# ironhide23586/RoomNet

Hardware: AMD Instinct MI355X
Metric: images/sec, 224x224 batch-256 RoomNet inference (higher is better)
Workload: dtype bf16; 1 GPU; RoomNet forward (reference final_model weights), uint8 BGR 224x224x3 in HBM -> probs+ids in HBM, batch 256 per GPU, bf16 storage / fp32 accumulate; images_per_gpu=256, global_batch=256, im_side=224, parallelism=dp1

## Files before the change

roomnet_amd/csrc/rn_stage4x.hip:

```cpp
#include "rn_fused.h"
#include "rn_stage.h"

#include <utility>

using namespace rnk;

namespace {

constexpr int U_NS = 4;
constexpr int U_AHEAD = 3;
constexpr int U_RINGPX = 208;
constexpr int U_ROW = U_RINGPX * 64;
constexpr int U_TAB_BYTES = 4 * 64 * 4;
constexpr int U_RING_OFF = U_TAB_BYTES;
constexpr int U_LDS = U_RING_OFF + U_NS * U_ROW;
constexpr int U_WMIN = 193, U_WMAX = 206;

template <int DT, int NQ>
__global__ __launch_bounds__(NQ == 4 ? 512 : 768, NQ == 4 ? 2 : 3) void stage4x_kernel(const StageArgs a) {
    constexpr int U_NW = NQ == 4 ? 8 : 12;
    constexpr int U_NTH = U_NW * 64;
    constexpr int U_NT = NQ == 4 ? 7 : 4;
    constexpr int U_NU = (U_NT + 1) / 2;
    RN_CLOCK_ENTRY();
    extern __shared__ __attribute__((aligned(64))) char smem[];
    const int tid = threadIdx.x;
    const int lane = tid & 63;
    const int wave = __builtin_amdgcn_readfirstlane(tid >> 6);
    const int cq = NQ == 4 ? (wave & 3) : (wave >> 2);
    const int run = NQ == 4 ? (wave >> 2) : (((wave & 3) + (wave >> 2)) & 3);
    const int px16 = lane & 15, g = lane >> 4;
    const int cb = blockIdx.x % a.n_cb, band = blockIdx.x / a.n_cb, n = blockIdx.y;
    const int Win = a.W, Wo_full = a.Wo, Ho = a.Ho;
    const int xo0 = a.cb_xo0[cb], Wo = a.cb_wo[cb];
    const int x0 = 2 * xo0;
    const int W = min(2 * Wo + 4, Win - x0);
    const int yo0 = band * a.rows_per_band;
    const int nrows = min(Ho, yo0 + a.rows_per_band) - yo0;
    const int y0 = 2 * yo0;
    const int nconv = 2 * (nrows - 1) + 4;
    const int nin = nconv + 2;
    const f32x4 zero4 = {0.f, 0.f, 0.f, 0.f};
    constexpr int OOB = 0x40000000;

    char* const ring = smem + U_RING_OFF;
    const unsigned ring_lds = lds_addr(ring);
    for (int i = tid; i < U_NS * (U_RINGPX - U_WMIN) * 4; i += U_NTH) {
        const int slot = i / ((U_RINGPX - U_WMIN) * 4), rest = i % ((U_RINGPX - U_WMIN) * 4);
        const int p = U_WMIN + rest / 4, c = rest % 4;
        if (p >= W) *reinterpret_cast<i32x4*>(ring + slot * U_ROW + p * 64 + c * 16) = i32x4{0, 0, 0, 0};
    }

    const bool has7 = run == 0;
    const int xo_run = NQ == 4 ? (run ? 55 : 0) : (run ? 8 + 23 * run : 0);
    const int xw = 2 * xo_run;
    const int nout_run = NQ == 4 ? (has7 ? 55 : 47) : (has7 ? 31 : 23);

    i32x4 wf[9];
#pragma unroll
    for (int f = 0; f < 9; ++f) {
        const i32x4* src = a.wfrag + (f * 4 + cq) * 64 + lane;
        asm volatile("global_load_dwordx4 %0, %1, off" : "=v"(wf[f]) : "v"(src) : "memory");
    }

    const char* const in_img = reinterpret_cast<const char*>(a.in + static_cast<int64_t>(n) * Win * Win * 32) + x0 * 64;
    const int row_bytes = Win * 64;
    const unsigned goff0 = static_cast<unsigned>((tid >> 2) * 64 + (((tid & 3) ^ swz4x(tid >> 2)) << 4));
    const int tail_total = W * 4 - U_NTH;
    const int tailn = (tail_total + U_NW - 1) / U_NW;
    const int tail_start = min(wave * tailn, tail_total - 1);
    const int tail_cnt = max(1, min(tail_total - wave * tailn, tailn));
    const unsigned long long tail_mask = (1ull << tail_cnt) - 1ull;
    unsigned goff1;
    {
        const int q = U_NTH + tail_start + min(lane, tail_cnt - 1);
        const int p = q >> 2, c = q & 3;
        goff1 = static_cast<unsigned>(p * 64 + ((c ^ swz4x(p)) << 4));
    }
    auto issue_row = [&](int y, int slot) __attribute__((always_inline)) {
        const char* row = in_img + static_cast<int64_t>(y0 + min(y, nin - 1)) * row_bytes;
        unsigned o0 = goff0, o1 = goff1;
        asm volatile("" : "+v"(o0), "+v"(o1));
        dma16(row + o0, ring + slot * U_ROW + wave * 1024);
        dma16_masked(row + o1, ring + slot * U_ROW + (U_NTH + tail_start) * 16, tail_mask);
    };

    unsigned base[3];
#pragma unroll
    for (int kx = 0; kx < 3; ++kx) {
        const int p = xw + px16 + kx;
        base[kx] = ring_lds + static_cast<unsigned>(p * 64 + ((g ^ swz4x(p)) << 4));
    }

    RN_POOL_BANDS_S2(pmA, pmB, pmC, px16, g);

    int voff[U_NU];
#pragma unroll
    for (int u = 0; u < U_NU; ++u) {
        const int xo = xo_run + 16 * u + px16;
        const bool valid = 16 * u + px16 < nout_run && xo < Wo;
        voff[u] = valid ? ((xo0 + xo) * 64 + 16 * cq + 4 * g) * 2 : OOB;
    }
    [[maybe_unused]] i32x2 cq3v = {0, 0};
    if constexpr (NQ == 3) cq3v = *reinterpret_cast<const i32x2*>(a.cvals + 4 * g);
    const f32x4 sc = *reinterpret_cast<const f32x4*>(a.ptab + 16 * cq + 4 * g);
    const f32x4 sh = *reinterpret_cast<const f32x4*>(a.ptab + 64 + 16 * cq + 4 * g);

    f32x4 acc[3][U_NT];
    int hp[U_NT][2], pp2[U_NT][2];
#pragma unroll
    for (int k = 0; k < U_NT; ++k) {
        hp[k][0] = hp[k][1] = pp2[k][0] = pp2[k][1] = 0;
#pragma unroll
        for (int r3 = 0; r3 < 3; ++r3) acc[r3][k] = zero4;
    }
    const int out_row_bytes = Wo_full * 128;
    const char* const out_img = reinterpret_cast<const char*>(a.out + static_cast<int64_t>(n) * Ho * Wo_full * 64);

#pragma unroll
    for (int j = 0; j < U_AHEAD; ++j) issue_row(j, j);
    wait_vmcnt<0>();
#pragma unroll
    for (int f = 0; f < 9; ++f) asm volatile("" : "+v"(wf[f]));
    lds_barrier();

    int slot_cur = 0;
    i32x4 fq[2][3];
    auto reads_at = [&](auto KC, const unsigned (&bcr)[3]) __attribute__((always_inline)) {
        constexpr int k = decltype(KC)::value;
        auto& dst = fq[k & 1];
#pragma unroll
        for (int f = 0; f < 3; ++f) asm volatile("ds_read_b128 %0, %1 offset:%2" : "=v"(dst[f]) : "v"(bcr[f]), "n"(k * 1024));
    };
    {
        unsigned bc0[3] = {base[0], base[1], base[2]};
        reads_at(IC<0>{}, bc0);
    }
    auto step = [&](auto RC, auto PARC, int s) __attribute__((always_inline)) {
        constexpr int R = decltype(RC)::value, PAR = decltype(PARC)::value;
        constexpr int iN = R, iM = (R + 2) % 3, iO = (R + 1) % 3;
        wait_vmcnt<(NQ == 4 ? 5 : 4)>();
        raw_barrier();
        const unsigned so = static_cast<unsigned>(slot_cur * U_ROW);
        unsigned bc[3];
#pragma unroll
        for (int kx = 0; kx < 3; ++kx) bc[kx] = base[kx] + so;
        i32x4 op[U_NT + 1];
        op[U_NT - 1] = op[U_NT] = i32x4{0, 0, 0, 0};
        auto reads = [&](auto KC) __attribute__((always_inline)) { reads_at(KC, bc); };
        auto tile = [&](auto KC, auto NEXTC) __attribute__((always_inline)) {
            constexpr int k = decltype(KC)::value;
            constexpr bool NEXT = decltype(NEXTC)::value != 0;
            if constexpr (NEXT) reads(IC<k + 1>{});
            auto& cur = fq[k & 1];
            [&]<int... F>(std::integer_sequence<int, F...>) {
                (([&] {
                     asm volatile("s_waitcnt lgkmcnt(%1)" : "+v"(cur[F]) : "n"((NEXT ? 3 : 0) + 2 - F));
                     acc[iN][k] = mfma16<DT>(cur[F], wf[0 * 3 + F], F == 0 ? zero4 : acc[iN][k]);
                     acc[iM][k] = mfma16<DT>(cur[F], wf[1 * 3 + F], acc[iM][k]);
                     acc[iO][k] = mfma16<DT>(cur[F], wf[2 * 3 + F], acc[iO][k]);
                     if constexpr (k == 0 && F == 0) {
                         int sl = slot_cur + U_AHEAD;
                         sl = sl >= U_NS ? sl - U_NS : sl;
                         issue_row(s + U_AHEAD, sl);
                     }
                 }()),
                 ...);
            }(std::make_integer_sequence<int, 3>{});
            const f32x4 v = acc[iO][k];
            const int v0 = static_cast<int>(pack2_relu6_sixth(v[0], v[1]));
            const int v1 = static_cast<int>(pack2_relu6_sixth(v[2], v[3]));
            if constexpr (PAR == 0) {
                hp[k][0] = v0;
                hp[k][1] = v1;
            } else {
                const int n0 = pk_add_f16(hp[k][0], v0), n1 = pk_add_f16(hp[k][1], v1);
                op[k] = i32x4{pp2[k][0], pp2[k][1], n0, n1};
                pp2[k][0] = n0;
                pp2[k][1] = n1;
            }
        };
        [&]<int... K>(std::integer_sequence<int, K...>) {
            (tile(IC<K>{}, IC<(K + 2 < U_NT ? 1 : 0)>{}), ...);
        }(std::make_integer_sequence<int, U_NT - 1>{});
        if (has7) {
            reads(IC<U_NT - 1>{});
            tile(IC<U_NT - 1>{}, IC<0>{});
        }
        if constexpr (PAR == 1) {
            const int r = (s - 5) >> 1;
            const bool emit = s >= 5 && r < nrows;
            const int rr = min(max(r, 0), nrows - 1);
            const char* orow = out_img + static_cast<int64_t>(yo0 + rr) * out_row_bytes;
            const __amdgpu_buffer_rsrc_t rs = __builtin_amdgcn_make_buffer_rsrc(const_cast<char*>(orow), 0, out_row_bytes, 0x00020000);
            const int emask = emit ? 0 : OOB;
            [[maybe_unused]] const unsigned seed = (!a.dither || cq == a.plain_q) ? RN_SEED_PLAIN : rn_dither_seed(yo0 + rr);
            auto out = [&](auto UC) __attribute__((always_inline)) {
                constexpr int u = decltype(UC)::value;
                f32x4 H = mfma16<RN_DTYPE_F16>(op[2 * u], pmA, zero4);
                H = mfma16<RN_DTYPE_F16>(op[2 * u + 1], pmB, H);
                if constexpr (2 * u + 2 < U_NT) H = mfma16<RN_DTYPE_F16>(op[2 * u + 2], pmC, H);
                float y[4];
#pragma unroll
                for (int i = 0; i < 4; ++i) y[i] = __builtin_fmaf(H[i], sc[i], sh[i]);
                i32x2 d;
                if constexpr (DT == RN_DTYPE_BF16)
                    d = i32x2{static_cast<int>(pack2_sr_bf16(y[0], y[1], seed)), static_cast<int>(pack2_sr_bf16(y[2], y[3], seed))};
                else
                    d = i32x2{static_cast<int>(pack2<DT>(y[0], y[1])), static_cast<int>(pack2<DT>(y[2], y[3]))};
                __builtin_amdgcn_raw_buffer_store_b64(d, rs, voff[u] | emask, 0, 0);
                if constexpr (NQ == 3)
                    if (cq == 2) __builtin_amdgcn_raw_buffer_store_b64(cq3v, rs, (voff[u] + 32) | emask, 0, 0);
            };
            if constexpr (NQ == 4) {
                out(IC<0>{});
                out(IC<1>{});
                out(IC<2>{});
                if (has7) out(IC<3>{});
            } else {
                out(IC<0>{});
                out(IC<1>{});
            }
        }
        slot_cur = slot_cur == U_NS - 1 ? 0 : slot_cur + 1;
        asm volatile("s_waitcnt lgkmcnt(0)" ::: "memory");
        {
            const unsigned sn = static_cast<unsigned>(slot_cur * U_ROW);
            unsigned bn[3];
#pragma unroll
            for (int kx = 0; kx < 3; ++kx) bn[kx] = base[kx] + sn;
            reads_at(IC<0>{}, bn);
        }
    };
    int s = 0;
    for (; s + 5 < nin; s += 6) {
        step(IC<0>{}, IC<0>{}, s);
        step(IC<1>{}, IC<1>{}, s + 1);
        step(IC<2>{}, IC<0>{}, s + 2);
        step(IC<0>{}, IC<1>{}, s + 3);
        step(IC<1>{}, IC<0>{}, s + 4);
        step(IC<2>{}, IC<1>{}, s + 5);
    }
    const int rem = nin - s;
    if (rem > 0) step(IC<0>{}, IC<0>{}, s);
    if (rem > 1) step(IC<1>{}, IC<1>{}, s + 1);
    if (rem > 2) step(IC<2>{}, IC<0>{}, s + 2);
    if (rem > 3) step(IC<0>{}, IC<1>{}, s + 3);
    if (rem > 4) step(IC<1>{}, IC<0>{}, s + 4);
    wait_vmcnt<0>();
    RN_CLOCK_EXIT(a.stamp_buf, threadIdx.x == 256);
}

}

bool rn_stage4x_plan(int out_side, int* n_cb, int* xo0, int* wo) {
    return rn_colblock_plan(out_side, (U_WMIN + 1 - 4 + 1) / 2, (U_WMAX - 4) / 2, n_cb, xo0, wo);
}

bool rn_stage4x_supported(int cin, int cout, int pool_k, int pool_s, bool res, int in_side) {
    int ncb, xo0[4], wo[4];
    return cin == 32 && cout == 64 && pool_k == 4 && pool_s == 2 && !res && in_side >= U_WMIN &&
           rn_stage4x_plan((in_side - 6) / 2 + 1, &ncb, xo0, wo);
}

void rn_stage4x_pack(const float* w_hwio, int dtype, std::vector<unsigned short>* out) {
    out->assign(static_cast<size_t>(9) * 4 * 64 * 8, 0);
    for (int f = 0; f < 9; ++f)
        for (int q = 0; q < 4; ++q)
            for (int l = 0; l < 64; ++l)
                for (int j = 0; j < 8; ++j) {
                    const int k = f * 32 + 8 * (l >> 4) + j, co = 16 * q + (l & 15);
                    const float v = w_hwio[static_cast<size_t>(k) * 64 + co];
                    (*out)[((static_cast<size_t>(f) * 4 + q) * 64 + l) * 8 + j] = rn_to16(v, dtype);
                }
}

int rn_stage4x_launch(int dtype, hipStream_t s, const StageArgs& a, int n) {
    int nthreads = 512;
    auto launch = [&]<auto Kern>(rn_kernel<Kern>) -> int {
        if (int rc = rn_allow_big_lds<Kern>()) return rc;
        hipLaunchKernelGGL(Kern, dim3(a.n_bands * a.n_cb, n), dim3(nthreads), U_LDS, s, a);
        RN_CHECK_LAUNCH();
        return RN_OK;
    };
    bool q3 = a.live_q == 3;
    for (int b = 0; b < a.n_cb; ++b) q3 = q3 && a.cb_wo[b] <= 100;
    if (q3) {
        nthreads = 768;
        if (dtype == RN_DTYPE_BF16) return launch(rn_kernel<stage4x_kernel<RN_DTYPE_BF16, 3>>{});
        return launch(rn_kernel<stage4x_kernel<RN_DTYPE_F16, 3>>{});
    }
    if (dtype == RN_DTYPE_BF16) return launch(rn_kernel<stage4x_kernel<RN_DTYPE_BF16, 4>>{});
    return launch(rn_kernel<stage4x_kernel<RN_DTYPE_F16, 4>>{});
}
```

roomnet_amd/csrc/rn_stage5x.hip:

```cpp
#include "rn_fused.h"
#include "rn_stage.h"

#include <utility>

using namespace rnk;

namespace {

constexpr int V_NS = 9;
constexpr int V_AHEAD = 3;
constexpr int V_RINGPX = 112;
constexpr int V_ROW = V_RINGPX * 128;
constexpr int V_TAB_BYTES = 4 * 64 * 4;
constexpr int V_RING_OFF = V_TAB_BYTES;
constexpr int V_LDS = V_RING_OFF + V_NS * V_ROW;
constexpr int V_WMIN = 66, V_WMAX = 110;
static_assert(V_LDS <= 160 * 1024, "LDS budget");

template <int DT, bool K48>
__global__ __launch_bounds__(512, 2) void stage5x_kernel(const StageArgs a) {
    constexpr int NF = K48 ? 5 : 6;
    RN_CLOCK_ENTRY();
    extern __shared__ __attribute__((aligned(64))) char smem[];
    const int tid = threadIdx.x;
    const int lane = tid & 63;
    const int wave = __builtin_amdgcn_readfirstlane(tid >> 6);
    const bool fold = a.live_q == 2;
    const int cq = fold ? (wave < 4 ? (wave >> 1) : 2 + ((wave - 4) >> 1)) : (wave & 3);
    const int ph = fold ? (wave & 1) : (wave >> 2);
    const bool conv_live = !fold || cq < 2;
    const bool epi_live = !K48 || cq < 3;
    const int px16 = lane & 15, g = lane >> 4;
    const int cb = blockIdx.x % a.n_cb, band = blockIdx.x / a.n_cb, n = blockIdx.y;
    const int Win = a.W, Wo_full = a.Wo, Ho = a.Ho;
    const int xo0 = a.cb_xo0[cb], Wo = a.cb_wo[cb];
    const int x0 = 2 * xo0;
    const int W = min(2 * Wo + 6, Win - x0);
    const int yo0 = band * a.rows_per_band;
    const int nrows = min(Ho, yo0 + a.rows_per_band) - yo0;
    const int y0 = 2 * yo0;
    const int nconv = 2 * (nrows - 1) + 4;
    const int nin = nconv + 2;
    const f32x4 zero4 = {0.f, 0.f, 0.f, 0.f};
    constexpr int OOB = 0x40000000;

    float* const tab = reinterpret_cast<float*>(smem);
    if (tid < 256) tab[tid] = a.ptab[tid];
    char* const ring = smem + V_RING_OFF;
    const unsigned ring_lds = lds_addr(ring);
    for (int i = tid; i < V_NS * (V_RINGPX - V_WMIN) * 8; i += 512) {
        const int slot = i / ((V_RINGPX - V_WMIN) * 8), rest = i % ((V_RINGPX - V_WMIN) * 8);
        const int p = V_WMIN + rest / 8, c = rest % 8;
        if (p >= W) *reinterpret_cast<i32x4*>(ring + slot * V_ROW + p * 128 + c * 16) = i32x4{0, 0, 0, 0};
    }

    const bool has4 = ph == 0;
    const int xw = ph ? 62 : 0;
    const int xo_run = ph ? 31 : 0;
    const int nout_run = has4 ? 31 : 23;

    i32x4 wf[3 * NF];
#pragma unroll
    for (int f = 0; f < 3 * NF; ++f) {
        const i32x4* src = a.wfrag + (f * 4 + cq) * 64 + lane;
        asm volatile("global_load_dwordx4 %0, %1, off" : "=v"(wf[f]) : "v"(src) : "memory");
    }

    const char* const in_img = reinterpret_cast<const char*>(a.in + static_cast<int64_t>(n) * Win * Win * 64) + x0 * 128;
    const int row_bytes = Win * 128;
    const unsigned goff0 = static_cast<unsigned>((tid >> 3) * 128 + (((tid & 7) ^ swz8(tid >> 3)) << 4));
    const int tailn = W - 64;
    const unsigned long long tail_mask = tailn >= 64 ? ~0ull : ((1ull << tailn) - 1ull);
    unsigned goff1;
    {
        const int q = 512 + wave * tailn + min(lane, tailn - 1);
        const int p = q >> 3, c = q & 7;
        goff1 = static_cast<unsigned>(p * 128 + ((c ^ swz8(p)) << 4));
    }
    auto issue_row = [&](int y, int slot) __attribute__((always_inline)) {
        const char* row = in_img + static_cast<int64_t>(y0 + min(y, nin - 1)) * row_bytes;
        unsigned o0 = goff0, o1 = goff1;
        asm volatile("" : "+v"(o0), "+v"(o1));
        dma16(row + o0, ring + slot * V_ROW + wave * 1024);
        dma16_masked(row + o1, ring + slot * V_ROW + (512 + wave * tailn) * 16, tail_mask);
    };

    unsigned base[3][2];
#pragma unroll
    for (int kx = 0; kx < 3; ++kx)
#pragma unroll
        for (int ch = 0; ch < 2; ++ch) {
            const int p = xw + px16 + kx;
            base[kx][ch] = ring_lds + static_cast<unsigned>(p * 128 + (((4 * ch + g) ^ swz8(p)) << 4));
        }
    if constexpr (K48) {
#pragma unroll
        for (int j = 0; j < 2; ++j) {
            const int p = xw + px16 + (j == 0 ? (g >> 1) : 2);
            base[j][1] = ring_lds + static_cast<unsigned>(p * 128 + (((4 + (g & 1)) ^ swz8(p)) << 4));
        }
    }

    RN_POOL_BANDS_S2(pmA, pmB, pmC, px16, g);

    unsigned a_tr[2][2][2];
    i32x4 wx[2][2];
    int voff[2];
    {
        const int q = px16 >> 2, pp = px16 & 3;
#pragma unroll
        for (int u = 0; u < 2; ++u) {
            const int xo_first = min(xo_run + 16 * u, Wo - 1);
            const int xs_u = min(a.rlo[xo0 + xo_first] - x0, W - 64);
            const int xo = xo_run + 16 * u + px16;
            const bool valid = 16 * u + px16 < nout_run && xo < Wo;
            voff[u] = valid ? ((xo0 + xo) * 64 + 16 * cq + 4 * g) * 2 : OOB;
            const int xq = xo0 + min(xo, Wo - 1);
            const int plo = a.rlo[xq] - x0, phi = a.rhi[xq] - x0;
            const float xlq = res_quant_lerp<DT>(a.rlerp[xq]);
#pragma unroll
            for (int kh = 0; kh < 2; ++kh) {
                unsigned short wh[8];
#pragma unroll
                for (int j = 0; j < 8; ++j) {
                    const int xin = xs_u + 32 * kh + 4 * g + 16 * (j >> 2) + (j & 3);
                    float w = 0.f;
                    if (xin == plo) w += 1.0f - xlq;
                    if (xin == phi) w += xlq;
                    wh[j] = to16<DT>(w);
                }
#pragma unroll
                for (int d = 0; d < 4; ++d) wx[u][kh][d] = static_cast<int>(static_cast<unsigned>(wh[2 * d]) | (static_cast<unsigned>(wh[2 * d + 1]) << 16));
#pragma unroll
                for (int t2 = 0; t2 < 2; ++t2) {
                    const int pix = xs_u + 32 * kh + 4 * g + 16 * t2 + q;
                    const int chunk = 2 * cq + (pp >> 1);
                    a_tr[u][kh][t2] = ring_lds + static_cast<unsigned>(pix * 128 + ((chunk ^ swz8(pix)) << 4) + (pp & 1) * 8);
                }
            }
        }
    }
    asm volatile("" : "+v"(wx[0][0]), "+v"(wx[0][1]), "+v"(wx[1][0]), "+v"(wx[1][1]));
    const f32x4 sc1 = *reinterpret_cast<const f32x4*>(a.ptab + 16 * cq + 4 * g);
    const f32x4 sh1 = *reinterpret_cast<const f32x4*>(a.ptab + 64 + 16 * cq + 4 * g);
    const f32x4 sc2 = *reinterpret_cast<const f32x4*>(a.ptab + 128 + 16 * cq + 4 * g);

    f32x4 acc[3][4];
    int hp[4][2], pp2[4][2];
#pragma unroll
    for (int k = 0; k < 4; ++k) {
        hp[k][0] = hp[k][1] = pp2[k][0] = pp2[k][1] = 0;
#pragma unroll
        for (int r3 = 0; r3 < 3; ++r3) acc[r3][k] = zero4;
    }
    const int out_row_bytes = Wo_full * 128;
    const char* const out_img = reinterpret_cast<const char*>(a.out + static_cast<int64_t>(n) * Ho * Wo_full * 64);

#pragma unroll
    for (int j = 0; j < V_AHEAD; ++j) issue_row(j, j);
    wait_vmcnt<0>();
#pragma unroll
    for (int f = 0; f < 3 * NF; ++f) asm volatile("" : "+v"(wf[f]));
    f32x4 cst4 = zero4;
    if constexpr (K48) {
        const float c0 = a.cstart[16 * cq + px16];
        cst4 = f32x4{c0, c0, c0, c0};
    }
    lds_barrier();

    int slot_cur = 0;
    auto step = [&](auto RC, auto PARC, int s) __attribute__((always_inline)) {
        constexpr int R = decltype(RC)::value, PAR = decltype(PARC)::value;
        constexpr int iN = R, iM = (R + 2) % 3, iO = (R + 1) % 3;
        wait_vmcnt<PAR == 0 ? 8 : 6>();
        raw_barrier();
        {
            int sl = slot_cur + V_AHEAD;
            sl = sl >= V_NS ? sl - V_NS : sl;
            issue_row(s + V_AHEAD, sl);
        }
        const unsigned so = static_cast<unsigned>(slot_cur * V_ROW);
        unsigned bc[3][2];
#pragma unroll
        for (int kx = 0; kx < 3; ++kx)
#pragma unroll
            for (int ch = 0; ch < 2; ++ch) bc[kx][ch] = base[kx][ch] + so;
        i32x4 fq[2][3];
        auto reads = [&](auto BC) __attribute__((always_inline)) {
            constexpr int b = decltype(BC)::value, k = b >> 1, ch = b & 1;
            constexpr int NR = (K48 && ch) ? 2 : 3;
            auto& dst = fq[b & 1];
            auto& bcr = bc;
#pragma unroll
            for (int kx = 0; kx < NR; ++kx) asm volatile("ds_read_b128 %0, %1 offset:%2" : "=v"(dst[kx]) : "v"(bcr[kx][ch]), "n"(k * 2048));
        };
        auto batch = [&](auto BC, auto NEXTC) __attribute__((always_inline)) {
            constexpr int b = decltype(BC)::value, k = b >> 1, ch = b & 1;
            constexpr bool NEXT = decltype(NEXTC)::value != 0;
            constexpr int NR = (K48 && ch) ? 2 : 3;
            constexpr int NRN = NEXT ? ((K48 && !ch) ? 2 : 3) : 0;
            if constexpr (NEXT) reads(IC<b + 1>{});
            auto& cur = fq[b & 1];
            [&]<int... KX>(std::integer_sequence<int, KX...>) {
                (([&] {
                     constexpr int fi = K48 ? (ch ? 3 + KX : KX) : KX * 2 + ch;
                     asm volatile("s_waitcnt lgkmcnt(%1)" : "+v"(cur[KX]) : "n"(NRN + NR - 1 - KX));
                     acc[iN][k] = mfma16<DT>(cur[KX], wf[0 * NF + fi], (ch == 0 && KX == 0) ? cst4 : acc[iN][k]);
                     acc[iM][k] = mfma16<DT>(cur[KX], wf[1 * NF + fi], acc[iM][k]);
                     acc[iO][k] = mfma16<DT>(cur[KX], wf[2 * NF + fi], acc[iO][k]);
                 }()),
                 ...);
            }(std::make_integer_sequence<int, NR>{});
        };
        auto tile = [&](auto KC, auto LASTC) __attribute__((always_inline)) {
            constexpr int k = decltype(KC)::value;
            constexpr bool LAST = decltype(LASTC)::value != 0;
            batch(IC<2 * k>{}, IC<1>{});
            batch(IC<2 * k + 1>{}, IC<(LAST ? 0 : 1)>{});
        };
        i32x4 op[4];
        op[3] = i32x4{0, 0, 0, 0};
        auto finish = [&](auto KC) __attribute__((always_inline)) {
            constexpr int k = decltype(KC)::value;
            const f32x4 v = acc[iO][k];
            const int v0 = static_cast<int>(pack2_relu6_sixth(v[0], v[1]));
            const int v1 = static_cast<int>(pack2_relu6_sixth(v[2], v[3]));
            if constexpr (PAR == 0) {
                hp[k][0] = v0;
                hp[k][1] = v1;
            } else {
                const int n0 = pk_add_f16(hp[k][0], v0), n1 = pk_add_f16(hp[k][1], v1);
                op[k] = i32x4{pp2[k][0], pp2[k][1], n0, n1};
                pp2[k][0] = n0;
                pp2[k][1] = n1;
            }
        };
        i32x4 fq5[2][K48 ? 5 : 1];
        auto reads5 = [&](auto KC) __attribute__((always_inline)) {
            constexpr int k = decltype(KC)::value;
            auto& dst = fq5[k & 1];
            auto& bcr = bc;
#pragma unroll
            for (int f = 0; f < 5; ++f) asm volatile("ds_read_b128 %0, %1 offset:%2" : "=v"(dst[f]) : "v"(f < 3 ? bcr[f][0] : bcr[f - 3][1]), "n"(k * 2048));
        };
        auto tile5 = [&](auto KC, auto NEXTC) __attribute__((always_inline)) {
            constexpr int k = decltype(KC)::value;
            constexpr bool NEXT = decltype(NEXTC)::value != 0;
            if constexpr (NEXT) reads5(IC<k + 1>{});
            auto& cur = fq5[k & 1];
            [&]<int... F>(std::integer_sequence<int, F...>) {
                (([&] {
                     asm volatile("s_waitcnt lgkmcnt(%1)" : "+v"(cur[F]) : "n"((NEXT ? 5 : 0) + 4 - F));
                     acc[iN][k] = mfma16<DT>(cur[F], wf[0 * NF + F], F == 0 ? cst4 : acc[iN][k]);
                     acc[iM][k] = mfma16<DT>(cur[F], wf[1 * NF + F], acc[iM][k]);
                     acc[iO][k] = mfma16<DT>(cur[F], wf[2 * NF + F], acc[iO][k]);
                 }()),
                 ...);
            }(std::make_integer_sequence<int, 5>{});
        };
        if constexpr (K48) {
            if (conv_live) {
                reads5(IC<0>{});
                tile5(IC<0>{}, IC<1>{});
                finish(IC<0>{});
                tile5(IC<1>{}, IC<1>{});
                finish(IC<1>{});
                tile5(IC<2>{}, IC<0>{});
                finish(IC<2>{});
                if (has4) {
                    reads5(IC<3>{});
                    tile5(IC<3>{}, IC<0>{});
                    finish(IC<3>{});
                }
            }
        } else
        if (conv_live) {
            reads(IC<0>{});
            tile(IC<0>{}, IC<0>{});
            finish(IC<0>{});
            tile(IC<1>{}, IC<0>{});
            finish(IC<1>{});
            tile(IC<2>{}, IC<1>{});
            finish(IC<2>{});
            if (has4) {
                reads(IC<6>{});
                tile(IC<3>{}, IC<1>{});
                finish(IC<3>{});
            }
        }
        if constexpr (PAR == 1) {
            const int r = (s - 5) >> 1;
            const bool emit = s >= 5 && r < nrows;
            const int rr = min(max(r, 0), nrows - 1);
            const float src = mul_rounded(static_cast<float>(yo0 + rr), a.rscale);
            const int ylo_v = static_cast<int>(src);
            const int ylo = __builtin_amdgcn_readfirstlane(ylo_v);
            const float yl = __int_as_float(__builtin_amdgcn_readfirstlane(__float_as_int(src - static_cast<float>(ylo_v))));
            const int yhi = min(ylo + 1, Win - 1);
            int dlo = s - (ylo - y0), dhi = s - (yhi - y0);
            dlo = min(max(dlo, 0), V_NS - 1);
            dhi = min(max(dhi, 0), V_NS - 1);
            int slo = slot_cur - dlo, shi = slot_cur - dhi;
            slo = slo < 0 ? slo + V_NS : slo;
            shi = shi < 0 ? shi + V_NS : shi;
            const unsigned olo = static_cast<unsigned>(slo * V_ROW), ohi = static_cast<unsigned>(shi * V_ROW);
            const char* orow = out_img + static_cast<int64_t>(yo0 + rr) * out_row_bytes;
            const __amdgpu_buffer_rsrc_t rs = __builtin_amdgcn_make_buffer_rsrc(const_cast<char*>(orow), 0, out_row_bytes, 0x00020000);
            const int emask = emit ? 0 : OOB;
            [[maybe_unused]] const unsigned seed = (!a.dither || cq == a.plain_q) ? RN_SEED_PLAIN : rn_dither_seed(yo0 + rr);
            if (!epi_live) {
                const i32x2 cv = *reinterpret_cast<const i32x2*>(a.cvals + 4 * g);
                __builtin_amdgcn_raw_buffer_store_b64(cv, rs, voff[0] | emask, 0, 0);
                __builtin_amdgcn_raw_buffer_store_b64(cv, rs, voff[1] | emask, 0, 0);
            } else
#pragma unroll
            for (int u = 0; u < 2; ++u) {
                i32x2 tq[2][2][2];
#pragma unroll
                for (int kh = 0; kh < 2; ++kh)
#pragma unroll
                    for (int t2 = 0; t2 < 2; ++t2) {
                        const unsigned alo = a_tr[u][kh][t2] + olo, ahi = a_tr[u][kh][t2] + ohi;
                        asm volatile("ds_read_b64_tr_b16 %0, %1" : "=v"(tq[0][kh][t2]) : "v"(alo));
                        asm volatile("ds_read_b64_tr_b16 %0, %1" : "=v"(tq[1][kh][t2]) : "v"(ahi));
                    }
                f32x4 H = zero4;
                if (conv_live) {
                    H = mfma16<RN_DTYPE_F16>(op[2 * u], pmA, zero4);
                    H = mfma16<RN_DTYPE_F16>(op[2 * u + 1], pmB, H);
                    if (u == 0) H = mfma16<RN_DTYPE_F16>(op[2], pmC, H);
                }
                asm volatile("s_waitcnt lgkmcnt(0)"
                             : "+v"(tq[0][0][0]), "+v"(tq[0][0][1]), "+v"(tq[0][1][0]), "+v"(tq[0][1][1]), "+v"(tq[1][0][0]), "+v"(tq[1][0][1]),
                               "+v"(tq[1][1][0]), "+v"(tq[1][1][1]));
                f32x4 r_lo = zero4, r_hi = zero4;
#pragma unroll
                for (int kh = 0; kh < 2; ++kh) {
                    const i32x4 al = {tq[0][kh][0][0], tq[0][kh][0][1], tq[0][kh][1][0], tq[0][kh][1][1]};
                    const i32x4 ah = {tq[1][kh][0][0], tq[1][kh][0][1], tq[1][kh][1][0], tq[1][kh][1][1]};
                    r_lo = mfma16<DT>(al, wx[u][kh], r_lo);
                    r_hi = mfma16<DT>(ah, wx[u][kh], r_hi);
                }
                float y[4];
#pragma unroll
                for (int i = 0; i < 4; ++i) {
                    const float y1 = __builtin_fmaf(H[i], sc1[i], sh1[i]);
                    const float lo = r_lo[i];
                    const float rsv = __builtin_fmaf(r_hi[i] - lo, yl, lo);
                    y[i] = __builtin_fmaf(rsv, sc2[i], y1);
                }
                i32x2 d;
                if constexpr (DT == RN_DTYPE_BF16)
                    d = i32x2{static_cast<int>(pack2_sr_bf16(y[0], y[1], seed)), static_cast<int>(pack2_sr_bf16(y[2], y[3], seed))};
                else
                    d = i32x2{static_cast<int>(pack2<DT>(y[0], y[1])), static_cast<int>(pack2<DT>(y[2], y[3]))};
                __builtin_amdgcn_raw_buffer_store_b64(d, rs, voff[u] | emask, 0, 0);
            }
        }
        slot_cur = slot_cur == V_NS - 1 ? 0 : slot_cur + 1;
        asm volatile("s_waitcnt lgkmcnt(0)" ::: "memory");
    };
    int s = 0;
    for (; s + 5 < nin; s += 6) {
        step(IC<0>{}, IC<0>{}, s);
        step(IC<1>{}, IC<1>{}, s + 1);
        step(IC<2>{}, IC<0>{}, s + 2);
        step(IC<0>{}, IC<1>{}, s + 3);
        step(IC<1>{}, IC<0>{}, s + 4);
        step(IC<2>{}, IC<1>{}, s + 5);
    }
    const int rem = nin - s;
    if (rem > 0) step(IC<0>{}, IC<0>{}, s);
    if (rem > 1) step(IC<1>{}, IC<1>{}, s + 1);
    if (rem > 2) step(IC<2>{}, IC<0>{}, s + 2);
    if (rem > 3) step(IC<0>{}, IC<1>{}, s + 3);
    if (rem > 4) step(IC<1>{}, IC<0>{}, s + 4);
    wait_vmcnt<0>();
    RN_CLOCK_EXIT(a.stamp_buf, threadIdx.x == 256);
}

}

bool rn_stage5x_plan(int out_side, int* n_cb, int* xo0, int* wo) {
    return rn_colblock_plan(out_side, (V_WMIN - 4 + 1) / 2, (V_WMAX - 4) / 2, n_cb, xo0, wo);
}

bool rn_stage5x_supported(int cin, int cout, int pool_k, int pool_s, bool res, int in_side, int skip_side) {
    int ncb, xo0[4], wo[4];
    const int out_side = (in_side - 6) / 2 + 1;
    return cin == 64 && cout == 64 && pool_k == 4 && pool_s == 2 && res && in_side >= V_WMIN && skip_side == in_side &&
           in_side - 2 * out_side <= 5 && rn_stage5x_plan(out_side, &ncb, xo0, wo);
}

void rn_stage5x_pack(const float* w_hwio, int dtype, std::vector<unsigned short>* out) {
    out->assign(static_cast<size_t>(18) * 4 * 64 * 8, 0);
    for (int f = 0; f < 18; ++f)
        for (int q = 0; q < 4; ++q)
            for (int l = 0; l < 64; ++l)
                for (int j = 0; j < 8; ++j) {
                    const int tap = f >> 1, ch = f & 1;
                    const int k = tap * 64 + 32 * ch + 8 * (l >> 4) + j, co = 16 * q + (l & 15);
                    const float v = w_hwio[static_cast<size_t>(k) * 64 + co];
                    (*out)[((static_cast<size_t>(f) * 4 + q) * 64 + l) * 8 + j] = rn_to16(v, dtype);
                }
}

void rn_stage5x_pack48(const float* w_hwio, int dtype, std::vector<unsigned short>* out) {
    out->assign(static_cast<size_t>(15) * 4 * 64 * 8, 0);
    for (int ky = 0; ky < 3; ++ky)
        for (int j = 0; j < 5; ++j)
            for (int q = 0; q < 4; ++q)
                for (int l = 0; l < 64; ++l)
                    for (int e = 0; e < 8; ++e) {
                        const int g = l >> 4, co = 16 * q + (l & 15);
                        int kx, ch;
                        if (j < 3) {
                            kx = j;
                            ch = 8 * g + e;
                        } else if (j == 3) {
                            kx = g >> 1;
                            ch = 32 + 8 * (g & 1) + e;
                        } else {
                            if (g >= 2) continue;
                            kx = 2;
                            ch = 32 + 8 * g + e;
                        }
                        const float v = w_hwio[(static_cast<size_t>(ky * 3 + kx) * 64 + ch) * 64 + co];
                        (*out)[((static_cast<size_t>(ky * 5 + j) * 4 + q) * 64 + l) * 8 + e] = rn_to16(v, dtype);
                    }
}

int rn_stage5x_launch(int dtype, hipStream_t s, const StageArgs& a, int n) {
    auto launch = [&]<auto Kern>(rn_kernel<Kern>) -> int {
        if (int rc = rn_allow_big_lds<Kern>()) return rc;
        hipLaunchKernelGGL(Kern, dim3(a.n_bands * a.n_cb, n), dim3(512), V_LDS, s, a);
        RN_CHECK_LAUNCH();
        return RN_OK;
    };
    if (a.cstart && a.live_q == 2) {
        if (dtype == RN_DTYPE_BF16) return launch(rn_kernel<stage5x_kernel<RN_DTYPE_BF16, true>>{});
        return launch(rn_kernel<stage5x_kernel<RN_DTYPE_F16, true>>{});
    }
    if (dtype == RN_DTYPE_BF16) return launch(rn_kernel<stage5x_kernel<RN_DTYPE_BF16, false>>{});
    return launch(rn_kernel<stage5x_kernel<RN_DTYPE_F16, false>>{});
}
```

Baseline: 242,900 images/sec.

## Specialize stage4x/5x row loops with compile-time slots and incremental row pointers

Both fused stage kernels get a restructured row loop. Ring slot indices become compile-time constants, so LDS reads use immediate offsets. Input and output row pointers advance incrementally instead of being recomputed from the step index. The runtime branches has7/has4/conv_live/epi_live are hoisted into template-specialized steady-state loops, and the per-row dither seeds are precomputed. The aim is to cut scalar and vector address arithmetic and branch overhead in the inner loop, at the cost of larger code and a subtle early-row masking scheme (early/early_adv) that must reproduce the old emit logic exactly.

```diff
diff --git a/roomnet_amd/csrc/rn_stage4x.hip b/roomnet_amd/csrc/rn_stage4x.hip
--- a/roomnet_amd/csrc/rn_stage4x.hip
+++ b/roomnet_amd/csrc/rn_stage4x.hip
@@ -77,8 +77,8 @@
         const int p = q >> 2, c = q & 3;
         goff1 = static_cast<unsigned>(p * 64 + ((c ^ swz4x(p)) << 4));
     }
-    auto issue_row = [&](int y, int slot) __attribute__((always_inline)) {
-        const char* row = in_img + static_cast<int64_t>(y0 + min(y, nin - 1)) * row_bytes;
+    auto issue_row = [&](const char* row, auto SLOTC) __attribute__((always_inline)) {
+        constexpr int slot = decltype(SLOTC)::value;
         unsigned o0 = goff0, o1 = goff1;
         asm volatile("" : "+v"(o0), "+v"(o1));
         dma16(row + o0, ring + slot * U_ROW + wave * 1024);
@@ -117,41 +117,42 @@
     const int out_row_bytes = Wo_full * 128;
     const char* const out_img = reinterpret_cast<const char*>(a.out + static_cast<int64_t>(n) * Ho * Wo_full * 64);
 
-#pragma unroll
-    for (int j = 0; j < U_AHEAD; ++j) issue_row(j, j);
+    const char* in_row = in_img + static_cast<int64_t>(y0) * row_bytes;
+    issue_row(in_row, IC<0>{});
+    issue_row(in_row + row_bytes, IC<1>{});
+    issue_row(in_row + 2 * static_cast<int64_t>(row_bytes), IC<2>{});
+    in_row += 3 * static_cast<int64_t>(row_bytes);
+    const char* orow = out_img + static_cast<int64_t>(yo0) * out_row_bytes;
+    [[maybe_unused]] unsigned sd[3];
+#pragma unroll
+    for (int t = 0; t < 3; ++t) sd[t] = (!a.dither || cq == a.plain_q) ? RN_SEED_PLAIN : rn_dither_seed(yo0 + t + 1);
     wait_vmcnt<0>();
 #pragma unroll
     for (int f = 0; f < 9; ++f) asm volatile("" : "+v"(wf[f]));
     lds_barrier();
 
-    int slot_cur = 0;
     i32x4 fq[2][3];
-    auto reads_at = [&](auto KC, const unsigned (&bcr)[3]) __attribute__((always_inline)) {
-        constexpr int k = decltype(KC)::value;
+    auto reads_at = [&](auto KC, auto SLOTC) __attribute__((always_inline)) {
+        constexpr int k = decltype(KC)::value, slot = decltype(SLOTC)::value;
         auto& dst = fq[k & 1];
-#pragma unroll
-        for (int f = 0; f < 3; ++f) asm volatile("ds_read_b128 %0, %1 offset:%2" : "=v"(dst[f]) : "v"(bcr[f]), "n"(k * 1024));
-    };
-    {
-        unsigned bc0[3] = {base[0], base[1], base[2]};
-        reads_at(IC<0>{}, bc0);
-    }
-    auto step = [&](auto RC, auto PARC, int s) __attribute__((always_inline)) {
-        constexpr int R = decltype(RC)::value, PAR = decltype(PARC)::value;
+        auto& bcr = base;
+#pragma unroll
+        for (int f = 0; f < 3; ++f) asm volatile("ds_read_b128 %0, %1 offset:%2" : "=v"(dst[f]) : "v"(bcr[f]), "n"(slot * U_ROW + k * 1024));
+    };
+    auto step = [&](auto IDXC, auto H7C, unsigned in_adv, int early, unsigned early_adv) __attribute__((always_inline)) {
+        constexpr int I = decltype(IDXC)::value, R = I % 3, PAR = I % 2, SLOT = I % 4;
+        constexpr bool H7 = decltype(H7C)::value != 0;
+        constexpr int NTW = H7 ? U_NT : U_NT - 1;
         constexpr int iN = R, iM = (R + 2) % 3, iO = (R + 1) % 3;
         wait_vmcnt<(NQ == 4 ? 5 : 4)>();
         raw_barrier();
-        const unsigned so = static_cast<unsigned>(slot_cur * U_ROW);
-        unsigned bc[3];
-#pragma unroll
-        for (int kx = 0; kx < 3; ++kx) bc[kx] = base[kx] + so;
+        __builtin_amdgcn_sched_barrier(0);
         i32x4 op[U_NT + 1];
         op[U_NT - 1] = op[U_NT] = i32x4{0, 0, 0, 0};
-        auto reads = [&](auto KC) __attribute__((always_inline)) { reads_at(KC, bc); };
         auto tile = [&](auto KC, auto NEXTC) __attribute__((always_inline)) {
             constexpr int k = decltype(KC)::value;
             constexpr bool NEXT = decltype(NEXTC)::value != 0;
-            if constexpr (NEXT) reads(IC<k + 1>{});
+            if constexpr (NEXT) reads_at(IC<k + 1>{}, IC<SLOT>{});
             auto& cur = fq[k & 1];
             [&]<int... F>(std::integer_sequence<int, F...>) {
                 (([&] {
@@ -160,9 +161,8 @@
                      acc[iM][k] = mfma16<DT>(cur[F], wf[1 * 3 + F], acc[iM][k]);
                      acc[iO][k] = mfma16<DT>(cur[F], wf[2 * 3 + F], acc[iO][k]);
                      if constexpr (k == 0 && F == 0) {
-                         int sl = slot_cur + U_AHEAD;
-                         sl = sl >= U_NS ? sl - U_NS : sl;
-                         issue_row(s + U_AHEAD, sl);
+                         issue_row(in_row, IC<(SLOT + U_AHEAD) % U_NS>{});
+                         in_row += in_adv;
                      }
                  }()),
                  ...);
@@ -181,20 +181,12 @@
             }
         };
         [&]<int... K>(std::integer_sequence<int, K...>) {
-            (tile(IC<K>{}, IC<(K + 2 < U_NT ? 1 : 0)>{}), ...);
-        }(std::make_integer_sequence<int, U_NT - 1>{});
-        if (has7) {
-            reads(IC<U_NT - 1>{});
-            tile(IC<U_NT - 1>{}, IC<0>{});
-        }
+            (tile(IC<K>{}, IC<(K + 1 < NTW ? 1 : 0)>{}), ...);
+        }(std::make_integer_sequence<int, NTW>{});
         if constexpr (PAR == 1) {
-            const int r = (s - 5) >> 1;
-            const bool emit = s >= 5 && r < nrows;
-            const int rr = min(max(r, 0), nrows - 1);
-            const char* orow = out_img + static_cast<int64_t>(yo0 + rr) * out_row_bytes;
             const __amdgpu_buffer_rsrc_t rs = __builtin_amdgcn_make_buffer_rsrc(const_cast<char*>(orow), 0, out_row_bytes, 0x00020000);
-            const int emask = emit ? 0 : OOB;
-            [[maybe_unused]] const unsigned seed = (!a.dither || cq == a.plain_q) ? RN_SEED_PLAIN : rn_dither_seed(yo0 + rr);
+            constexpr bool EARLY = I == 1 || I == 3;
+            [[maybe_unused]] const unsigned seed = sd[((I - 1) / 2) % 3];
             auto out = [&](auto UC) __attribute__((always_inline)) {
                 constexpr int u = decltype(UC)::value;
                 f32x4 H = mfma16<RN_DTYPE_F16>(op[2 * u], pmA, zero4);
@@ -208,45 +200,52 @@
                     d = i32x2{static_cast<int>(pack2_sr_bf16(y[0], y[1], seed)), static_cast<int>(pack2_sr_bf16(y[2], y[3], seed))};
                 else
                     d = i32x2{static_cast<int>(pack2<DT>(y[0], y[1])), static_cast<int>(pack2<DT>(y[2], y[3]))};
-                __builtin_amdgcn_raw_buffer_store_b64(d, rs, voff[u] | emask, 0, 0);
+                const int vo = EARLY ? (voff[u] | early) : voff[u];
+                __builtin_amdgcn_raw_buffer_store_b64(d, rs, vo, 0, 0);
                 if constexpr (NQ == 3)
-                    if (cq == 2) __builtin_amdgcn_raw_buffer_store_b64(cq3v, rs, (voff[u] + 32) | emask, 0, 0);
+                    if (cq == 2) __builtin_amdgcn_raw_buffer_store_b64(cq3v, rs, EARLY ? ((voff[u] + 32) | early) : voff[u] + 32, 0, 0);
             };
             if constexpr (NQ == 4) {
                 out(IC<0>{});
                 out(IC<1>{});
                 out(IC<2>{});
-                if (has7) out(IC<3>{});
+                if constexpr (H7) out(IC<3>{});
             } else {
                 out(IC<0>{});
                 out(IC<1>{});
             }
+            orow += EARLY ? early_adv : static_cast<unsigned>(out_row_bytes);
         }
-        slot_cur = slot_cur == U_NS - 1 ? 0 : slot_cur + 1;
         asm volatile("s_waitcnt lgkmcnt(0)" ::: "memory");
-        {
-            const unsigned sn = static_cast<unsigned>(slot_cur * U_ROW);
-            unsigned bn[3];
-#pragma unroll
-            for (int kx = 0; kx < 3; ++kx) bn[kx] = base[kx] + sn;
-            reads_at(IC<0>{}, bn);
+        reads_at(IC<0>{}, IC<(SLOT + 1) % U_NS>{});
+    };
+    auto steady = [&](auto H7C) __attribute__((always_inline)) {
+        reads_at(IC<0>{}, IC<0>{});
+        int left = nin;
+        int early = OOB;
+        unsigned early_adv = 0;
+        for (;;) {
+            bool done = false;
+            [&]<int... P>(std::integer_sequence<int, P...>) {
+                (([&] {
+                     if (done) return;
+                     const unsigned in_adv = left >= 6 ? static_cast<unsigned>(row_bytes) : 0u;
+                     step(IC<2 * P>{}, H7C, in_adv, early, early_adv);
+                     step(IC<2 * P + 1>{}, H7C, in_adv, early, early_adv);
+                     left -= 2;
+                     done = left == 0;
+                 }()),
+                 ...);
+            }(std::make_integer_sequence<int, 6>{});
+            if (done) break;
+            early = 0;
+            early_adv = static_cast<unsigned>(out_row_bytes);
         }
     };
-    int s = 0;
-    for (; s + 5 < nin; s += 6) {
-        step(IC<0>{}, IC<0>{}, s);
-        step(IC<1>{}, IC<1>{}, s + 1);
-        step(IC<2>{}, IC<0>{}, s + 2);
-        step(IC<0>{}, IC<1>{}, s + 3);
-        step(IC<1>{}, IC<0>{}, s + 4);
-        step(IC<2>{}, IC<1>{}, s + 5);
-    }
-    const int rem = nin - s;
-    if (rem > 0) step(IC<0>{}, IC<0>{}, s);
-    if (rem > 1) step(IC<1>{}, IC<1>{}, s + 1);
-    if (rem > 2) step(IC<2>{}, IC<0>{}, s + 2);
-    if (rem > 3) step(IC<0>{}, IC<1>{}, s + 3);
-    if (rem > 4) step(IC<1>{}, IC<0>{}, s + 4);
+    if (has7)
+        steady(IC<1>{});
+    else
+        steady(IC<0>{});
     wait_vmcnt<0>();
     RN_CLOCK_EXIT(a.stamp_buf, threadIdx.x == 256);
 }
diff --git a/roomnet_amd/csrc/rn_stage5x.hip b/roomnet_amd/csrc/rn_stage5x.hip
--- a/roomnet_amd/csrc/rn_stage5x.hip
+++ b/roomnet_amd/csrc/rn_stage5x.hip
@@ -77,12 +77,11 @@
         const int p = q >> 3, c = q & 7;
         goff1 = static_cast<unsigned>(p * 128 + ((c ^ swz8(p)) << 4));
     }
-    auto issue_row = [&](int y, int slot) __attribute__((always_inline)) {
-        const char* row = in_img + static_cast<int64_t>(y0 + min(y, nin - 1)) * row_bytes;
+    auto issue_row = [&](const char* row, int slot_off) __attribute__((always_inline)) {
         unsigned o0 = goff0, o1 = goff1;
         asm volatile("" : "+v"(o0), "+v"(o1));
-        dma16(row + o0, ring + slot * V_ROW + wave * 1024);
-        dma16_masked(row + o1, ring + slot * V_ROW + (512 + wave * tailn) * 16, tail_mask);
+        dma16(row + o0, ring + slot_off + wave * 1024);
+        dma16_masked(row + o1, ring + slot_off + (512 + wave * tailn) * 16, tail_mask);
     };
 
     unsigned base[3][2];
@@ -156,8 +155,16 @@
     const int out_row_bytes = Wo_full * 128;
     const char* const out_img = reinterpret_cast<const char*>(a.out + static_cast<int64_t>(n) * Ho * Wo_full * 64);
 
-#pragma unroll
-    for (int j = 0; j < V_AHEAD; ++j) issue_row(j, j);
+    const char* in_row = in_img + static_cast<int64_t>(y0) * row_bytes;
+    issue_row(in_row, 0);
+    issue_row(in_row + row_bytes, V_ROW);
+    issue_row(in_row + 2 * static_cast<int64_t>(row_bytes), 2 * V_ROW);
+    in_row += 3 * static_cast<int64_t>(row_bytes);
+    const char* orow = out_img + static_cast<int64_t>(yo0) * out_row_bytes;
+    int rr = 0;
+    [[maybe_unused]] unsigned sd[3];
+#pragma unroll
+    for (int t = 0; t < 3; ++t) sd[t] = (!a.dither || cq == a.plain_q) ? RN_SEED_PLAIN : rn_dither_seed(yo0 + t + 1);
     wait_vmcnt<0>();
 #pragma unroll
     for (int f = 0; f < 3 * NF; ++f) asm volatile("" : "+v"(wf[f]));
@@ -169,17 +176,18 @@
     lds_barrier();
 
     int slot_cur = 0;
-    auto step = [&](auto RC, auto PARC, int s) __attribute__((always_inline)) {
-        constexpr int R = decltype(RC)::value, PAR = decltype(PARC)::value;
+    int so_cur = 0, sl_cur = V_AHEAD * V_ROW;
+    int s = 0;
+    auto step = [&](auto IDXC, auto CLC, auto H4C, auto ELC, unsigned in_adv, int early, int early_adv) __attribute__((always_inline)) {
+        constexpr int I = decltype(IDXC)::value, R = I % 3, PAR = I % 2;
+        constexpr bool CL = decltype(CLC)::value != 0, H4 = decltype(H4C)::value != 0, EL = decltype(ELC)::value != 0;
         constexpr int iN = R, iM = (R + 2) % 3, iO = (R + 1) % 3;
         wait_vmcnt<PAR == 0 ? 8 : 6>();
         raw_barrier();
-        {
-            int sl = slot_cur + V_AHEAD;
-            sl = sl >= V_NS ? sl - V_NS : sl;
-            issue_row(s + V_AHEAD, sl);
-        }
-        const unsigned so = static_cast<unsigned>(slot_cur * V_ROW);
+        issue_row(in_row, sl_cur);
+        in_row += in_adv;
+        sl_cur = sl_cur == (V_NS - 1) * V_ROW ? 0 : sl_cur + V_ROW;
+        const unsigned so = static_cast<unsigned>(so_cur);
         unsigned bc[3][2];
 #pragma unroll
         for (int kx = 0; kx < 3; ++kx)
@@ -258,40 +266,33 @@
                  ...);
             }(std::make_integer_sequence<int, 5>{});
         };
-        if constexpr (K48) {
-            if (conv_live) {
-                reads5(IC<0>{});
-                tile5(IC<0>{}, IC<1>{});
-                finish(IC<0>{});
-                tile5(IC<1>{}, IC<1>{});
-                finish(IC<1>{});
-                tile5(IC<2>{}, IC<0>{});
-                finish(IC<2>{});
-                if (has4) {
-                    reads5(IC<3>{});
-                    tile5(IC<3>{}, IC<0>{});
-                    finish(IC<3>{});
-                }
+        if constexpr (K48 && CL) {
+            reads5(IC<0>{});
+            tile5(IC<0>{}, IC<1>{});
+            finish(IC<0>{});
+            tile5(IC<1>{}, IC<1>{});
+            finish(IC<1>{});
+            tile5(IC<2>{}, IC<(H4 ? 1 : 0)>{});
+            finish(IC<2>{});
+            if constexpr (H4) {
+                tile5(IC<3>{}, IC<0>{});
+                finish(IC<3>{});
             }
-        } else
-        if (conv_live) {
+        } else if constexpr (CL) {
             reads(IC<0>{});
             tile(IC<0>{}, IC<0>{});
             finish(IC<0>{});
             tile(IC<1>{}, IC<0>{});
             finish(IC<1>{});
-            tile(IC<2>{}, IC<1>{});
+            tile(IC<2>{}, IC<(H4 ? 0 : 1)>{});
             finish(IC<2>{});
-            if (has4) {
-                reads(IC<6>{});
+            if constexpr (H4) {
                 tile(IC<3>{}, IC<1>{});
                 finish(IC<3>{});
             }
         }
         if constexpr (PAR == 1) {
-            const int r = (s - 5) >> 1;
-            const bool emit = s >= 5 && r < nrows;
-            const int rr = min(max(r, 0), nrows - 1);
+            constexpr bool EARLY = I == 1 || I == 3;
             const float src = mul_rounded(static_cast<float>(yo0 + rr), a.rscale);
             const int ylo_v = static_cast<int>(src);
             const int ylo = __builtin_amdgcn_readfirstlane(ylo_v);
@@ -304,11 +305,10 @@
             slo = slo < 0 ? slo + V_NS : slo;
             shi = shi < 0 ? shi + V_NS : shi;
             const unsigned olo = static_cast<unsigned>(slo * V_ROW), ohi = static_cast<unsigned>(shi * V_ROW);
-            const char* orow = out_img + static_cast<int64_t>(yo0 + rr) * out_row_bytes;
             const __amdgpu_buffer_rsrc_t rs = __builtin_amdgcn_make_buffer_rsrc(const_cast<char*>(orow), 0, out_row_bytes, 0x00020000);
-            const int emask = emit ? 0 : OOB;
-            [[maybe_unused]] const unsigned seed = (!a.dither || cq == a.plain_q) ? RN_SEED_PLAIN : rn_dither_seed(yo0 + rr);
-            if (!epi_live) {
+            const int emask = EARLY ? early : 0;
+            [[maybe_unused]] const unsigned seed = sd[((I - 1) / 2) % 3];
+            if constexpr (!EL) {
                 const i32x2 cv = *reinterpret_cast<const i32x2*>(a.cvals + 4 * g);
                 __builtin_amdgcn_raw_buffer_store_b64(cv, rs, voff[0] | emask, 0, 0);
                 __builtin_amdgcn_raw_buffer_store_b64(cv, rs, voff[1] | emask, 0, 0);
@@ -325,7 +325,7 @@
                         asm volatile("ds_read_b64_tr_b16 %0, %1" : "=v"(tq[1][kh][t2]) : "v"(ahi));
                     }
                 f32x4 H = zero4;
-                if (conv_live) {
+                if constexpr (CL) {
                     H = mfma16<RN_DTYPE_F16>(op[2 * u], pmA, zero4);
                     H = mfma16<RN_DTYPE_F16>(op[2 * u + 1], pmB, H);
                     if (u == 0) H = mfma16<RN_DTYPE_F16>(op[2], pmC, H);
@@ -356,25 +356,47 @@
                     d = i32x2{static_cast<int>(pack2<DT>(y[0], y[1])), static_cast<int>(pack2<DT>(y[2], y[3]))};
                 __builtin_amdgcn_raw_buffer_store_b64(d, rs, voff[u] | emask, 0, 0);
             }
+            const int adv = EARLY ? early_adv : 1;
+            rr += adv;
+            orow += static_cast<unsigned>(adv ? out_row_bytes : 0);
         }
         slot_cur = slot_cur == V_NS - 1 ? 0 : slot_cur + 1;
+        so_cur = so_cur == (V_NS - 1) * V_ROW ? 0 : so_cur + V_ROW;
+        ++s;
         asm volatile("s_waitcnt lgkmcnt(0)" ::: "memory");
     };
-    int s = 0;
-    for (; s + 5 < nin; s += 6) {
-        step(IC<0>{}, IC<0>{}, s);
-        step(IC<1>{}, IC<1>{}, s + 1);
-        step(IC<2>{}, IC<0>{}, s + 2);
-        step(IC<0>{}, IC<1>{}, s + 3);
-        step(IC<1>{}, IC<0>{}, s + 4);
-        step(IC<2>{}, IC<1>{}, s + 5);
-    }
-    const int rem = nin - s;
-    if (rem > 0) step(IC<0>{}, IC<0>{}, s);
-    if (rem > 1) step(IC<1>{}, IC<1>{}, s + 1);
-    if (rem > 2) step(IC<2>{}, IC<0>{}, s + 2);
-    if (rem > 3) step(IC<0>{}, IC<1>{}, s + 3);
-    if (rem > 4) step(IC<1>{}, IC<0>{}, s + 4);
+    auto steady = [&](auto CLC, auto H4C, auto ELC) __attribute__((always_inline)) {
+        int left = nin;
+        int early = OOB, early_adv = 0;
+#pragma nounroll
+        for (;;) {
+            bool done = false;
+            [&]<int... P>(std::integer_sequence<int, P...>) {
+                (([&] {
+                     if (done) return;
+                     const unsigned in_adv = left >= 6 ? static_cast<unsigned>(row_bytes) : 0u;
+                     step(IC<2 * P>{}, CLC, H4C, ELC, in_adv, early, early_adv);
+                     step(IC<2 * P + 1>{}, CLC, H4C, ELC, in_adv, early, early_adv);
+                     left -= 2;
+                     done = left == 0;
+                 }()),
+                 ...);
+            }(std::make_integer_sequence<int, 3>{});
+            if (done) break;
+            early = 0;
+            early_adv = 1;
+        }
+    };
+    if (conv_live) {
+        if (has4)
+            steady(IC<1>{}, IC<1>{}, IC<1>{});
+        else
+            steady(IC<1>{}, IC<0>{}, IC<1>{});
+    } else if (epi_live) {
+        steady(IC<0>{}, IC<0>{}, IC<1>{});
+    } else {
+        steady(IC<0>{}, IC<0>{}, IC<0>{});
+    }
     wait_vmcnt<0>();
     RN_CLOCK_EXIT(a.stamp_buf, threadIdx.x == 256);
 }
```

New measurement: 246,400 images/sec (median of 6 runs). 1.01x the previous value.
